# sijieaaa/AGPlace

Measured on AMD Instinct MI355X. Metric: aerial-ground pairs/sec (backbone+ODE+pool), higher is better.
Workload: dtype f16 (fp16 x fp16, fp32 accumulate); 1 GPU; nuScenes-AG 6-cam (C3/C4): MM.forward_q on [b,3,224,1344] + DBVanilla2D on [b,1,3,224,224], ResNet18 stem+layer1-3, euler h=0.1 x3 FCODE, GeM, stage-2 fusion; inference forward; the voxel branch's pooled outputs enter as fixed tensors (SURVEY.md 8d); global_batch=64, parallelism=dp1, bn=per-rank (eval: running statistics), paired_trunks=True, hipgraph=True, steps_in_flight=2, library_default_precision=4, headline_is_library_default=True, streams=2, query_sub_batches_on_streams=1, query_input=fp32 normalised panorama

## Files before the change

### agplace_amd/_lib.py

```python
import ctypes as C
import os

_HERE = os.path.dirname(os.path.abspath(__file__))
LIB_PATH = os.environ.get("AGP_HIP_LIB") or os.path.join(_HERE, "lib", "libagplace_hip.so")

AGP_OK = 0
PREC_BF16 = 1
PREC_F16W2 = 2
PREC_BF16X3 = 3
PREC_F16 = 4
FMT_BF16, FMT_F16 = 0, 1
ACT = {None: 0, "id": 0, "relu": 1, "tanh": 2, "sigmoid": 3}
ODE = {"euler": 0, "midpoint": 1, "rk4": 2}
ODE_ADAPTIVE = {"dopri5": 3}
ODE_STATUS = {0: "ok", 1: "odeint_max_steps attempted steps did not reach t = 1", 2: "step size underflow (t + dt == t)",
              3: "the error ratio is NaN"}
ODE_MAX_STEPS_LIMIT = 4096
E_UNSUPPORTED = 3
GP_FLOATS = 1 + 16384 + 1
_ERR = {1: "AGP_E_BADARG (unsupported shape / enum / null pointer)",
        2: "AGP_E_LAUNCH (HIP launch failed)",
        3: "AGP_E_UNSUPPORTED"}


# ... 60 lines not shown
    "agp_resize_pack_u8_cams": (_I, [_P, _I, _I, _I, _I, _I, _I, _P, _P, _P, _P, C.POINTER(_F), C.POINTER(_F), _I, _P, _P, _P]),
    "agp_center_crop_origin": (_I, [_I, _I, _I, C.POINTER(_I), C.POINTER(_I)]),
    "agp_resize_u8_cams_roi": (_I, [_P, _I, _I, _L, _L, _I, _I, _I, _I, _I, _I, _P, _P, _P, _P, _P, _P]),
    "agp_resize_pack_u8_cams_roi": (_I, [_P, _I, _I, _L, _L, _I, _I, _I, _I, _I, _I, _P, _P, _P, _P, C.POINTER(_F), C.POINTER(_F), _I,
                                         _P, _P, _P]),
    "agp_jitter_u8_cams": (_I, [_P, _I, _I, _I, _I, _P, _P, _P, _P]),
    "agp_jitter_pack_u8_cams": (_I, [_P, _I, _I, _I, _I, _P, _P, C.POINTER(_F), C.POINTER(_F), _I, _P, _P, _P]),
    "agp_unpack_nhwc_to_f32": (_I, [_P, _P, _I, _I, _I, _I, _I, _P, _P]),
    "agp_map_zero_halo": (_I, [_P, _P, _I, _I, _I, _I, _I, _P]),
    "agp_map_absmax": (_I, [_P, _P, _I, _I, _I, _I, _I, _P, _P]),
    "agp_map_absmax_reset": (_I, [_P, _I, _P]),
    "agp_conv2d_fwd": (_I, [C.POINTER(ConvDesc), _P]),
    "agp_conv2d_fwd_grouped": (_I, [C.POINTER(ConvDesc), _I, _P]),
    "agp_conv2d_s2_fwd": (_I, [C.POINTER(ConvDesc), _I, _P]),
    "agp_conv2d_fwd_grouped2": (_I, [C.POINTER(ConvDesc), C.POINTER(ConvStream2), _I, _P]),
    "agp_bblock64_fwd_grouped": (_I, [C.POINTER(BBlock64Desc), _I, _P]),
    "agp_bblock64_pool_floats": (_L, [C.POINTER(BBlock64Desc)]),
    "agp_bblock64_pool_finish": (_I, [_P, _I, _I, _I, _P, _P]),
    "agp_conv_w_q8_prepare": (_I, [_P, _I, _I, _P, C.POINTER(C.c_int32), _P]),
    "agp_conv2d_tile_plan": (_I, [C.POINTER(ConvDesc), _I, C.POINTER(C.c_int32)]),
    "agp_conv2d_stat_tiles": (_I, [C.POINTER(ConvDesc)]),
    "agp_conv2d_pool_blocks": (_I, [C.POINTER(ConvDesc)]),
    "agp_pool_from_conv": (_I, [_P, _I, _I, _I, _I, _P, _P, _P, _P]),
    "agp_bn_stats_from_partial": (_I, [_P, _I, _I, _L, _F, _F, _P, _P, _P, _P, _P, _P, _P, _P, _P]),
    "agp_stem_pool_fwd": (_I, [C.POINTER(ConvDesc), _P]),
    "agp_stem_pool_raw_fwd": (_I, [C.POINTER(ConvDesc), _I, _L, _L, _L, _L, _I, C.POINTER(_F), C.POINTER(_F), _P]),
    "agp_maxpool3x3s2_fwd": (_I, [_P, _P, _I, _I, _I, _I, _I, _P, _P, _I, _I, _I, _P, _P]),
    "agp_bcast_add_fwd": (_I, [_P, _P, _P, _I, _I, _I, _I, _I, _P, _P, _I, _P]),
    "agp_pool_workspace_floats": (_L, [_I, _I, _I, _I]),
    "agp_pool_fwd": (_I, [_P, _P, _I, _I, _I, _I, _I, _P, _F, _P, _P, _P, _P]),
# ... 117 lines not shown
```

### agplace_amd/csrc/conv_dispatch.hip

```cpp
#include "conv_internal.hpp"
using namespace agp_igemm;

static bool fits_31(int n, int h, int w, int c) { return (int64_t)n * (h + 2) * (w + 2) * c * 2 < (1ll << 31); }

static bool conv_3x3s1(const agp_conv_desc* d) {
    return d->kh == 3 && d->kw == 3 && d->stride == 1 && d->pad == 1 && d->in_w_step == d->cin;
}
static bool conv_kxr_ok(const agp_conv_desc* d) {
    return conv_3x3s1(d) && d->pin == 1 && d->pout == 1 && d->hout == d->hin && d->wout == d->win && fits_31(d->n, d->hin, d->win, d->cin);
}

static bool kxr2_member_ok(const agp_conv_desc* d, const agp_conv_desc* d0) {
    return d->in_hi && d->w_hi && d->out_hi && !d->in_lo && !d->out_lo && !d->res_lo && d->n > 0 &&
           d->cin % 32 == 0 && d->cout % 64 == 0 && conv_kxr_ok(d) && agp_internal_use_kxr2(d) &&
           d->cin == d0->cin && d->cout == d0->cout;
}

static bool s2_conv_ok(const agp_conv_desc* c, const agp_conv_desc* d0) {
    return c->prec == AGP_PREC_F16 && c->in_hi && c->w_hi && c->out_hi && !c->in_lo && !c->out_lo && !c->res_hi &&
           !c->stat_partial && !c->pool_partial &&
           c->kh == 3 && c->kw == 3 && c->stride == 2 && c->pad == 1 && c->pin == 1 && c->pout == 1 && c->in_w_step == c->cin &&
           c->hout == (c->hin - 1) / 2 + 1 && c->wout == (c->win - 1) / 2 + 1 &&
           c->cin % 32 == 0 && c->cout % 64 == 0 && c->n > 0 && c->cin == d0->cin && c->cout == d0->cout &&
           fits_31(c->n, c->hin, c->win, c->cin) && fits_31(c->n, c->hout, c->wout, c->cout);
}
static bool s2_downsample_ok(const agp_conv_desc* d, const agp_conv_desc* c) {
    return d->prec == AGP_PREC_F16 && d->w_hi && d->out_hi && !d->in_lo && !d->out_lo && !d->res_hi && !d->stat_partial && !d->pool_partial &&
           d->kh == 1 && d->kw == 1 && d->stride == 2 && d->pad == 0 && d->pin == 1 && d->pout == 1 && d->in_w_step == d->cin &&
// ... 227 lines not shown
    KxrwStreams ds = {};
    const int rc = conv_fill_group(descs, n, ps, true);
    if (rc != AGP_OK) return rc;
    for (int i = 0; i < n; ++i) {
        const agp_conv_stream2* t = s2 + i;
        if (!t->in_hi) continue;
        const int wp = t->win + 2, hp = t->hin + 2;
        KxrwStream& k = ds.s[i];
        k.x = t->in_hi; k.w = t->w_cm;
        k.x_bytes = (uint32_t)((int64_t)t->n * hp * wp * t->cin * 2);
        k.w_bytes = (uint32_t)((int64_t)t->cin * descs[i].cout * 2);
        k.sn = hp * wp * t->cin; k.sh = 2 * wp * t->cin; k.sw = 2 * t->cin; k.base = (wp - 1) * t->cin;
        k.nc = t->cin / 32;
    }
    return agp_internal_conv_kxrw(ps, n, (hipStream_t)stream, nullptr, any ? &ds : nullptr);
}

static int stem_pool_impl(const agp_conv_desc* d, int kind, int64_t sn, int64_t sc, int64_t sh, int64_t sw, int ncam,
                          const float* mean3, const float* std3, void* stream) {
    if (!d || !d->in_hi || !d->w_hi || !d->out_hi || d->in_lo || d->out_lo || d->res_hi) return AGP_E_BADARG;
    if (d->prec != AGP_PREC_F16W2 && d->prec != AGP_PREC_F16) return AGP_E_BADARG;
    if (d->prec == AGP_PREC_F16W2 && !d->w_lo) return AGP_E_BADARG;
    if (d->cin != 32 || d->in_w_step != 4 || d->kw != 1 || d->kh != 7 || d->stride != 2 || d->pad != 3 || d->pin != 3 ||
        d->cout != 64 || !d->relu || d->n <= 0)
        return AGP_E_BADARG;
    const int h1 = (d->hin + 2 * 3 - 7) / 2 + 1, w1 = (d->win + 2 * 3 - 7) / 2 + 1;
    const int h2 = (h1 + 2 - 3) / 2 + 1, w2 = (w1 + 2 - 3) / 2 + 1;
    if (d->hout != h2 || d->wout != w2) return AGP_E_BADARG;
    IgemmParams p = {};
    const int hp = d->hin + 6, wp = d->win + 6;
// ... 30 lines not shown
```

### agplace_amd/csrc/igemm_kxrw.hip

```cpp

#include <type_traits>

#include "conv_internal.hpp"

namespace agp_igemm {

struct KxrwGroup {
    IgemmParams p[KXRW_MAXP];
    int mt_end[KXRW_MAXP];
    int nprob, MT, NT, mt_chunk;
    int MT_full, half_bid0;
    uint32_t* rflag;
    uint32_t r_bytes[KXRW_MAXP];
};
constexpr uint32_t KXRW_ROOB = 0xffffff00u;
__device__ __forceinline__ const KxrwStreams& kxrw_streams(const KxrwStreams& s) { return s; }

constexpr int KW_ROWB = 64;
template <int TM_, int TN_> struct KwShape {
    static constexpr int BM = 128 * TM_, BN = 32 * TN_, BMX = BM + 16;
    static constexpr int XBUF = BMX * KW_ROWB, WTAP = BN * KW_ROWB;
    static constexpr int LDS = 2 * XBUF + 3 * WTAP + 2 * BN * 4;
    static constexpr int STRIP = 32 * 2 * BN, XWAVES = XBUF / STRIP, SPARE = LDS + (TM_ == 1 ? 2048 : 0);
    static constexpr int EPI_LDS = SPARE + (4 - XWAVES) * STRIP;
// ... 397 lines not shown
#pragma unroll
                for (int e = 0; e < 8; ++e) v[e] += r[e];
            }
            rg.any8(v);
            outv[jj] = pack8_h_lo(v, relu_lo);
        }
#pragma unroll
        for (int jj = 0; jj < TN * 2; ++jj) *(u32x4*)(strip + a_off + ((jj ^ a_swz) << 5)) = outv[jj];
        __builtin_amdgcn_fence(__ATOMIC_RELEASE, "wavefront");
        u32x4 lines[NEI];
#pragma unroll
        for (int i = 0; i < NEI; ++i) lines[i] = *(const u32x4*)(strip + l_off + i * 1024);
        if constexpr (TM == 2) {
            if (tm == 0 && RES == 1) wait_vm_lgkm<0>();
        }
#pragma unroll
        for (int i = 0; i < NEI; ++i) {
            const int off = eoff[tm * NEI + i];
            if (off >= 0) *(u32x4*)(ohi + off) = lines[i];
        }
        if constexpr (POOL) {
            if (ppart) {
#pragma unroll
                for (int i = 0; i < NEI; ++i)
                    if (eoff[tm * NEI + i] < 0) *(u32x4*)(strip + l_off + i * 1024) = u32x4{0u, 0u, 0u, 0u};
                __builtin_amdgcn_fence(__ATOMIC_RELEASE, "wavefront");
                auto sweep = [&](auto STAT) {
#pragma clang fp contract(off)
                    constexpr int stat = decltype(STAT)::value;
#pragma unroll
                    for (int p8 = 0; p8 < 32; p8 += 8) {
                        uint32_t w[8];
#pragma unroll
                        for (int u = 0; u < 8; ++u) w[u] = *(const uint32_t*)(strip + (p8 + u) * (2 * BN) + ((lane * 4) ^ (((p8 + u) & 15) << 4)));
// ... 148 lines not shown
    return AGP_OK;
}

}

int agp_internal_conv_kxrw(agp_igemm::IgemmParams* ps, int n, hipStream_t s, agp_igemm::TilePlan* plan, const agp_igemm::KxrwStreams* ds) {
    using namespace agp_igemm;
    if (n < 1 || n > KXRW_MAXP || ps[0].N % 128) return AGP_E_BADARG;
    constexpr int bm = KwShape<2, 4>::BM, bn = KwShape<2, 4>::BN;
    KxrwGroup g = {};
    g.nprob = n;
    int mt = 0;
    bool pool = false;
    for (int i = 0; i < n; ++i) {
        if (ps[i].N != ps[0].N || ps[i].CK != ps[0].CK) return AGP_E_BADARG;
        g.p[i] = ps[i];
        mt += (ps[i].M + bm - 1) / bm;
        g.mt_end[i] = mt;
        pool = pool || ps[i].pool_partial != nullptr;
        const int64_t rb = (int64_t)(ps[i].M / (int)ps[i].d_howo.d) * ps[i].o_sn * 2;
        if (ps[i].r_hi && (rb <= 0 || rb > (int64_t)KXRW_ROOB)) return AGP_E_BADARG;
        g.r_bytes[i] = (uint32_t)rb;
    }
    g.MT = mt;
    g.NT = ps[0].N / bn;
    const KxrwPlan k = kxrw_plan(g.MT, g.NT);
    if (plan) {
        *plan = TilePlan{AGP_CONV_KERNEL_KXRW, bm, bn, g.MT, g.NT, k.MT_full, k.half_tiles, k.blocks};
        return AGP_OK;
    }
// ... 19 lines not shown
```

### agplace_amd/models_baseline/dbvanilla2d.py

```python
from typing import List

import torch
import torch.nn as nn

from .. import autograd_ops, ops, range_guard, train_fns
from ..network.image_fe import ImageFE
from ..network.image_pooling import GeM
from ..network_mm.ffns import _PreparedLinear
from ..options import get_options
from ..vecprog import VecProgram


class MLP(nn.Module):
    def __init__(self, input_dim, output_dim):
        super().__init__()
        self.seq = nn.Sequential(
            nn.Linear(input_dim, output_dim),
            nn.LayerNorm(output_dim),
            nn.ReLU(),
            nn.Linear(output_dim, output_dim),
        )
        self._p0, self._p3 = _PreparedLinear(self.seq[0]), _PreparedLinear(self.seq[3])

    def forward(self, x):
# ... 108 lines not shown
                    x = ops.RawFrames(f.reshape(b * ndb, 1, *f.shape[2:]), h, w, crop=crop,
                                      jitter=None if jitter is None else jitter[:, :, i].reshape(b * ndb, ops.JITTER_RECORD))
                else:
                    x = db_map[:, :, i].reshape(b * ndb, c, h, w)
                if u8:
                    x = x.permute(0, 2, 3, 1).unsqueeze(1)
                if train:
                    fe = self.dbimage_fes[j].fe
                    v = train_fns.TrunkFn.apply(train_fns.anchor_of(fe, self.dbimage_pools[j].p), x, fe, self.dbimage_pools[j], train_fns.MapSink(),
                                                prec, False, i if opt.share_dbfe is True else 0)[0]
                else:
                    if trunk_maps is not None and i in trunk_maps:
                        fpool = trunk_maps[i][1]
                    else:
                        fpool = self.final_pool_request(i)
                        self.dbimage_fes[j].forward_maps(x, prec=prec, final_pool=fpool)
                    v, vscale = (fpool.gem, fpool.scale) if fused is not None else (fpool.true_gem(), None)
                if fused is not None:
                    mlp = self.dbimage_mlps[j]
                    fused.linear(0, mlp._p0.get(), v, scale=vscale)
                    fused.layernorm(0, mlp.seq[1], 0, relu=True)
                    fused.linear(2 + i, mlp._p3.get(), 0)
                    if opt.output_l2 is True:
                        fused.l2norm(2 + i, 2 + i)
                    vecs.append(v)
                    continue
                v = self.dbimage_mlps[j](v)
                if opt.output_l2 is True:
                    v = autograd_ops.l2normalize(v)
                vecs.append(v)
            if fused is not None:
# ... 30 lines not shown
```

### agplace_amd/network_mm/image_fe.py

```python
import torch.nn as nn

from .. import range_guard
from ..options import get_options
from ..resnet import ResNet


class ImageFE(nn.Module):
    _ALLOWED = ("resnet18", "resnet34")
    _LAST_DIM = {"resnet18": {2: 128, 3: 256, 4: 512}, "resnet34": {2: 128, 3: 256, 4: 512},
                 "resnet50": {2: 512, 3: 1024, 4: 2048}}

    def __init__(self, fe_type, layers, opt=None):
        super().__init__()
        self.opt = opt
        self.fe_type = fe_type
        layers = [int(x) for x in layers.split('_')]
        self.layers = layers
        if fe_type not in self._ALLOWED or len(layers) not in (2, 3, 4):
            raise NotImplementedError
        self.last_dim = self._LAST_DIM[fe_type][len(layers)]
        self.fe = ResNet(fe_type, nstages=len(layers))

    def forward_maps(self, x, prec=None, level_means=None, final_pool=None):
        if len(self.layers) not in (3, 4):
            raise NotImplementedError
        prec = get_options().mfma_precision if prec is None else prec
        return self.fe.forward_maps(x, prec=prec, level_means=level_means, final_pool=final_pool)

    def export_precision(self):
        p = get_options().mfma_precision
        return 2 if p == 4 else p

    def forward(self, x, prec=None):
        prec = self.export_precision() if prec is None else prec
        with range_guard.guarded(self, self.opt or get_options(), prec, self.training):
            maps = self.forward_maps(x, prec=prec)
            x_list = [m.to_f32() for m in maps]
        return x_list[-1], x_list

    def poll_fp16_range(self):
        range_guard.poll(self)

# ... 3 lines not shown
```

### agplace_amd/network_mm/mm.py

```python
import torch
import torch.nn as nn

from .. import autograd_ops, ops, range_guard, sparse, train_fns
from ..options import get_options
from .ffns import _PreparedLinear
from .fuse_block_toshallow import FuseBlockToShallow
from ..vecprog import VecProgram, VecProgramUnfit
from .image_fe import ImageFE
from .image_pooling import GeM
from .stage2fuse_blockadd import Stage2FuseBlockAdd


class MM(nn.Module):
    def __init__(self, drop=None, opt=None):
        super().__init__()
        self.opt = opt = opt or get_options()
        self.drop = drop
        self.image_fe = ImageFE(fe_type=opt.mm_imgfe, layers=opt.mm_imgfe_layers)
        self.image_fe.fe.set_image_norm(opt.image_mean, opt.image_std)
        self.image_pool = GeM()
        planes = [int(x) for x in opt.mm_voxfe_planes.split('_')]
        layers = [int(x) for x in opt.mm_voxfe_layers.split('_')]
        self.vox_fe = sparse.MinkFPN(in_channels=1, out_channels=planes[-1], planes=planes, layers=layers,
                                     num_top_down=opt.mm_voxfe_ntd, conv0_kernel_size=5, block=sparse.ECABasicBlock)
# ... 294 lines not shown
            vp.linear(2, s2._prep_fuseimg[0].get(exp=-e3), 1)
            fv_img = vp.store(2)
        elif e3:
            vp.wsum(2, [1], [ops.pow2_scalar(dev, -e3)])
            fv_img = vp.store(2)
        if sparse_vox and s2._prep_fusevox[0] is not None:
            vp.linear(3, s2._prep_fusevox[0].get(), 1)
            fv_vox = vp.store(3)
        if rider and vp.fits_beside(rider[0]):
            vp.run(rider=rider.pop())
        else:
            vp.run()
        m = s2._ws.map("add0", imagefeatmap.n, imagefeatmap.h, imagefeatmap.w, imagefeatmap.c, 1, prec, dev)
        ops.bcast_add(imagefeatmap, fv_img, m)
        s2pool = ops.PoolReq(s2.poolimage.p, eps=s2.poolimage.eps, want_mean=True, want_gem=True, gem_out=out_rows.get('stg2imagevec'))
        imap = s2.ffnsimg[0].forward_map(m, prec, pool=s2pool)
        mean, stg2imagevec, s2scale = s2pool.mean, s2pool.gem, s2pool.scale
        if sparse_vox:
            vm = sparse.modules.seg_affine(voxmap, add=fv_vox)
            vm = s2.ffnsvox[0](vm, prec=prec)
            stg2voxvec = s2.poolvox(vm)
            vf = s2.projsvoxfuse[0][0](vm, prec=prec) if opt.stg2_useproj is True else vm
            voxvec_fuse = sparse.modules.global_avg_pool(vf)
        else:
            stg2voxvec, voxvec_fuse = data_dict['stg2voxvec'].float(), data_dict['voxvec_fuse'].float()
        vt = VecProgram(b, dev)
        if s2._prep_imgfuse[0] is not None:
            vt.linear(0, s2._prep_imgfuse[0].get(), mean, scale=s2scale)
        else:
            vt.load(0, mean, s2scale)
        vt.load(1, fusevec)
# ... 108 lines not shown
```

### agplace_amd/network_mm/stage2fuse_blockadd.py

```python
import torch
import torch.nn as nn

from .. import autograd_ops, ops, sparse, train_fns, train_graph
from ..options import get_options
from .ffns import _PreparedLinear
from .image_pooling import GeM


class _Conv1x1AsLinear:

    def __init__(self, conv):
        self.conv = conv

    @property
    def weight(self):
        return self.conv.weight.view(self.conv.out_channels, self.conv.in_channels)

    @property
    def bias(self):
        return self.conv.bias


class _PreparedConv1x1(_PreparedLinear):
    def __init__(self, conv):
# ... 23 lines not shown
        self._ws = ops.Workspace()
        self._units = None
        self._map_exp = {}

    def _prepared(self, e_io=0, e_mid=0):
        key = tuple((t.data_ptr(), t._version) for t in list(self.parameters()) + list(self.buffers())) + (e_io, e_mid)
        if key != self._key:
            cws = []
            for conv, bn, e_in, e_out in ((self.conv1, self.bn1, e_io, e_mid), (self.conv2, self.bn2, e_mid, e_io)):
                s, t = ops.fold_exp(*ops.fold_bn(bn.weight, bn.bias, bn.running_mean, bn.running_var, bn.eps,
                                                 conv_bias=conv.bias), e_in, e_out)
                cws.append(ops.ConvWeights(conv.weight, s, t, 1, 1))
            self._cw, self._key = cws, key
        return self._cw

    def forward_map(self, x: ops.SplitMap, prec=3, pool=None):
        e_mid = int(self._map_exp.get("conv1", 0)) if prec != 3 else 0
        c1, c2 = self._prepared(x.exp, e_mid)
        dev = x.hi.device
        t = self._ws.map("t", x.n, x.h, x.w, x.c, 1, prec, dev)
        o = self._ws.map("o", x.n, x.h, x.w, x.c, 1, prec, dev)
        t.exp, o.exp = e_mid, x.exp
        ops.probe_map(self, "in", x)
        ops.conv2d(x, c1, t, relu=True, prec=prec)
        ops.probe_map(self, "conv1", t)
        ops.conv2d(t, c2, o, residual=x, relu=True, prec=prec, pool=pool)
        ops.probe_map(self, "out", o)
        return o

    def forward(self, x, prec=3):
        if isinstance(x, ops.SplitMap):
            return self.forward_map(x, prec)
        xm = ops.pack_f32(x, x.shape[1], 1, prec)
        return self.forward_map(xm, prec).to_f32()

    def forward_map_train(self, x: ops.SplitMap, prec=3):
        if self._units is None:
# ... 169 lines not shown
```

### agplace_amd/ops.py

```python
import ctypes as C
import math
import os

import torch

from . import _lib
from ._lib import ptr, check

GEM_EPS = 1e-6
CONV_PROFILE = None
LO_FP8 = True
CHUNK_MAJOR_TRAIN = True
USE_W_CM = True


def _L():
    return _lib.load()


def _need_cuda(t, what):
    if not t.is_cuda:
        raise RuntimeError(f"{what}: tensor must live on the GPU (agplace_amd has no CPU path)")


# ... 87 lines not shown

def probe_map(owner, name, m):
    if MAP_PROBE is not None:
        MAP_PROBE(owner, name, m)


def map_absmax(m: SplitMap, word):
    check(_L().agp_map_absmax(ptr(m.hi), ptr(m.lo), m.n, m.h, m.w, m.c, m.pad, ptr(word), _lib.stream()), "agp_map_absmax")


def absmax_reset(words):
    check(_L().agp_map_absmax_reset(ptr(words), words.numel(), _lib.stream()), "agp_map_absmax_reset")


def count_saturated(m: SplitMap):
    if m.lo is not None:
        return 0
    return int((m.hi.view(torch.float16).abs() >= 65504).sum().item())


class Workspace:

    def __init__(self):
        self.bufs = {}

    def map(self, tag, n, h, w, c, pad, prec, device, h16=False):
        key = (tag, n, h, w, c, pad, prec, str(device), torch.cuda.current_stream(device).cuda_stream)
        m = self.bufs.get(key)
        if m is None:
            m = SplitMap.alloc(n, h, w, c, pad, prec, device)
            self.bufs[key] = m
# ... 437 lines not shown
    jobs = [tuple(j) + (None,) * (6 - len(j)) for j in jobs]
    arr = (_lib.ConvDesc * len(jobs))()
    for d, (x, cw, out, residual, relu, pool) in zip(arr, jobs):
        _fill_conv_desc(d, x, cw, out, residual, relu, prec)
        if pool is not None and x.lo is None and out.lo is None and int(_L().agp_conv2d_pool_blocks(C.byref(d))) > 0:
            d.pool_partial = 1
    if len(jobs) == 1:
        if stat_partial:
            arr[0].stat_partial = 1
        if hi_only:
            arr[0].hi_only = 1
        return tile_plan(arr[0])
    return tile_plan(arr)


class PoolReq:
    __slots__ = ("p", "eps", "want_mean", "want_gem", "mean", "gem", "fused", "_partial", "gem_out", "exp")

    def __init__(self, p=None, eps=GEM_EPS, want_mean=True, want_gem=False, gem_out=None):
        if want_gem and p is None:
            raise ValueError("PoolReq: GeM needs its exponent tensor p")
        self.p = None if p is None else p.detach()
        self.eps, self.want_mean, self.want_gem = eps, want_mean, want_gem
        self.mean = self.gem = self._partial = None
        self.gem_out = gem_out
        self.fused = False
        self.exp = 0

    @property
    def scale(self):
        t = self.mean if self.mean is not None else self.gem
        return pow2_scalar(t.device, self.exp)

    def true_mean(self):
        return scale_pow2(self.mean, self.exp)

    def true_gem(self):
        return scale_pow2(self.gem, self.exp)

    def attach(self, d, x, cw, out, prec):
        self.fused = False
        self.exp = out.exp
        if x.lo is None and out.lo is None:
            blocks = int(_L().agp_conv2d_pool_blocks(C.byref(d)))
            if blocks > 0:
                self._partial = torch.empty(blocks * 2 * cw.cout, dtype=torch.float32, device=out.hi.device)
                d.pool_partial = ptr(self._partial)
                d.pool_p = ptr(self.p) if self.want_gem else None
                d.pool_eps = math.ldexp(self.eps, -self.exp)
                self.fused = True

    def finish(self, out):
        go = self.gem_out
        if go is not None and (tuple(go.shape) != (out.n, out.c) or go.dtype != torch.float32 or not go.is_contiguous()):
            go = None
        self.exp = out.exp
        if not self.fused:
            self.mean, self.gem = pool_map(out, self.p, want_mean=self.want_mean, want_gem=self.want_gem, eps=self.eps, gem_out=go,
                                           raw=True)
            return
        dev = out.hi.device
        self.mean = torch.empty((out.n, out.c), dtype=torch.float32, device=dev) if self.want_mean else None
        self.gem = (go if go is not None else torch.empty((out.n, out.c), dtype=torch.float32, device=dev)) if self.want_gem else None
        check(_L().agp_pool_from_conv(ptr(self._partial), out.n, out.h, out.w, out.c, ptr(self.p) if self.want_gem else None,
                                      ptr(self.mean), ptr(self.gem), _lib.stream()), "agp_pool_from_conv")


class SqStatReq:
    __slots__ = ("fused", "partial", "blocks")

    def __init__(self):
        self.fused, self.partial, self.blocks = False, None, 0

    def attach(self, d, x, cw, out, prec):
        self.fused = False
        if x.lo is None and out.lo is None:
# ... 44 lines not shown
            if c2 is not None:
                d.w_cm, d.w_cm_lo = ptr(c2[0]), ptr(c2[1])
    if LO_FP8 and prec == _lib.PREC_F16W2:
        q = cw.q8()
        if q is not None:
            d.w_q8, d.w_q8_exp = ptr(q[0]), q[1]
    return d


def conv2d_grouped(jobs, prec):
    jobs = [tuple(j) + (None,) * (6 - len(j)) for j in jobs]
    if len(jobs) == 1:
        x, cw, out, residual, relu, pool = jobs[0]
        return [conv2d(x, cw, out, residual=residual, relu=relu, prec=prec, pool=pool)]
    arr = (_lib.ConvDesc * len(jobs))()
    keep = []
    for d, (x, cw, out, residual, relu, pool) in zip(arr, jobs):
        keep.append(cw.planes(prec))
        _fill_conv_desc(d, x, cw, out, residual, relu, prec)
        if pool is not None:
            pool.attach(d, x, cw, out, prec)
    e0 = e1 = None
    if CONV_PROFILE is not None:
        e0, e1 = torch.cuda.Event(enable_timing=True), torch.cuda.Event(enable_timing=True)
        e0.record()
    check(_L().agp_conv2d_fwd_grouped(arr, len(jobs), _lib.stream()), "agp_conv2d_fwd_grouped")
    if CONV_PROFILE is not None:
        e1.record()
        x, cw, out = jobs[0][:3]
        macs = sum(j[0].n * j[2].h * j[2].w * j[1].cout * j[1].alg_k for j in jobs)
        CONV_PROFILE.append((e0, e1, macs, (sum(j[0].n for j in jobs), out.h, out.w, cw.cin, cw.cout, cw.kh, cw.kw, cw.stride)))
    for j in jobs:
        if j[5] is not None:
            j[5].finish(j[2])
    return [j[2] for j in jobs]


class Stream2Weights:
    __slots__ = ("cin", "cout", "plane", "shift", "fusable")

    def __init__(self, weight, scale, shift):
# ... 29 lines not shown
            if x2.lo is not None or x2.pad != 1 or x2.c != sw.cin or sw.plane is None:
                raise ValueError("conv2d_grouped2: the second stream is a one-plane fp16 map with a 1-pixel halo and fusable weights")
            t.in_hi, t.w_cm = ptr(x2.hi), ptr(sw.plane)
            t.n, t.hin, t.win, t.cin = x2.n, x2.h, x2.w, sw.cin
    check(_L().agp_conv2d_fwd_grouped2(arr, st, len(jobs), _lib.stream()), "agp_conv2d_fwd_grouped2")
    return [j[2] for j in jobs]


def conv2d(x: SplitMap, cw: ConvWeights, out: SplitMap, residual: SplitMap = None, relu=False, prec=3, stat_partial=None, pool=None,
           bstat=None, hi_only=False):
    d = _fill_conv_desc(_lib.ConvDesc(), x, cw, out, residual, relu, prec, stat_partial, bstat)
    if hi_only:
        d.hi_only = 1
    if pool is not None:
        pool.attach(d, x, cw, out, prec)
    if CONV_PROFILE is not None:
        e0, e1 = torch.cuda.Event(enable_timing=True), torch.cuda.Event(enable_timing=True)
        e0.record()
        check(_L().agp_conv2d_fwd(C.byref(d), _lib.stream()), "agp_conv2d_fwd")
        e1.record()
        CONV_PROFILE.append((e0, e1, x.n * out.h * out.w * cw.cout * cw.alg_k,
                             (x.n, out.h, out.w, cw.cin, cw.cout, cw.kh, cw.kw, cw.stride)))
    else:
        check(_L().agp_conv2d_fwd(C.byref(d), _lib.stream()), "agp_conv2d_fwd")
    if pool is not None:
        pool.finish(out)
    return out


FUSED_BLOCK64 = True


def bblock64_ok(x: SplitMap, cw1: ConvWeights, cw2: ConvWeights, prec):
    if not FUSED_BLOCK64 or prec != _lib.PREC_F16 or x.lo is not None or x.pad != 1 or x.c != 64 or x.h % 2:
        return False
    for cw in (cw1, cw2):
        if (cw.cin, cw.cout, cw.kh, cw.kw, cw.stride, cw.pad) != (64, 64, 3, 3, 1, 1) or cw.in_w_step_stem or cw.w is None:
            return False
    return x.n * (x.h + 2) * (x.w + 2) * 128 < (1 << 31)
# ... 466 lines not shown
```

### agplace_amd/pair.py

```python
import torch


from . import ops, range_guard, resnet

RIDER = True


def can_pair(modelq, modeldb, qdata, dbdata):
    if modelq.training or modeldb.training or torch.is_grad_enabled():
        return False
    fq, fdbs = modelq.image_fe.fe, [m.fe for m in modeldb.dbimage_fes]
    db_map = dbdata['db_map']
    nmap = db_map.shape[-4]
    if modelq.opt.mfma_precision != modeldb.opt.mfma_precision or db_map.dim() not in (5, 6):
        return False
    if modeldb.opt.share_dbfe is True and nmap > 1:
        return False
    return all((f.fe_type, f.nstages) == (fq.fe_type, fq.nstages) for f in fdbs[:nmap])


def _resized_tiles(modelq, modeldb, qdata, dbdata):
    if 'query_jitter' in qdata and 'query_frames' not in qdata:
        raise ValueError("embed_pair: `query_jitter` (colour jitter records) needs `query_frames`")
    if 'db_jitter' in dbdata and 'db_frames' not in dbdata:
# ... 43 lines not shown
    b = img.shape[0]
    if k > 1 and 'coords' not in qdata and 'points' not in qdata and b % k == 0 and b >= 2 * k and db_map.shape[0] % k == 0:
        return _embed_pair_substreams(modelq, modeldb, qdata, dbdata, k)
    return _embed_pair_one(modelq, modeldb, qdata, dbdata)


def _embed_pair_one(modelq, modeldb, qdata, dbdata, q_rows=None, db_rows=None):
    opt = modelq.opt
    prec = opt.mfma_precision
    image = modelq.query_image(qdata)
    db_map = dbdata['db_map']
    u8 = db_map.dtype == torch.uint8
    if db_map.dim() == 5:
        db_map = db_map.unsqueeze(1)
    nets, xs, lms, fps = [modelq.image_fe.fe], [image], [[]], [modelq.final_pool_request()]
    nmap = db_map.shape[2]
    for i in range(nmap):
        nets.append(modeldb.dbimage_fes[i].fe)
        if u8:
            bb, ndb, _, h, w, _ = db_map.shape
            xs.append(db_map[:, :, i].reshape(bb * ndb, 1, h, w, 3))
        else:
            bb, ndb, _, c, h, w = db_map.shape
            xs.append(db_map[:, :, i].reshape(bb * ndb, c, h, w))
        lms.append(None)
        fps.append(modeldb.final_pool_request(i))
    maps = resnet.forward_maps_multi(nets, xs, prec=prec, level_means=lms, final_pools=fps)
    head = [] if RIDER else None
    out_db = modeldb.forward_db(dbdata, trunk_maps={i: (maps[1 + i], fps[1 + i]) for i in range(nmap)}, out_rows=db_rows,
                                defer_head=head)
    out_q = modelq.forward_q(qdata, image_maps=(maps[0], lms[0], fps[0]), out_rows=q_rows, rider=head)
    if head:
        head.pop().run()
    return out_q, out_db


def _slice(d, b, lo, hi):
    out = {}
    for name, v in d.items():
        if torch.is_tensor(v) and v.dim() > 0 and v.shape[0] == b:
            out[name] = v[lo:hi]
        elif isinstance(v, (list, tuple)) and all(torch.is_tensor(t) and t.shape[0] == b for t in v):
# ... 82 lines not shown
```

### agplace_amd/resnet.py

```python
import math

import os

import torch
import torch.nn as nn

from . import ops, train_graph

ARCH = {
    "resnet18": ("basic", [2, 2, 2, 2]),
    "resnet34": ("basic", [3, 4, 6, 3]),
    "resnet50": ("bottleneck", [3, 4, 6, 3]),
}
PLANES = [64, 128, 256, 512]


def _conv(cin, cout, k, stride, pad):
    m = nn.Conv2d(cin, cout, k, stride, pad, bias=False)
    nn.init.kaiming_normal_(m.weight, mode="fan_out", nonlinearity="relu")
    return m


class _Block(nn.Module):
    def __init__(self, kind, inplanes, planes, stride):
# ... 167 lines not shown
                raise ValueError("stem input map must be NHWC4 with halo 3 in the conv's storage format")
            return ops.slice_map(x, lo, hi)
        raw = isinstance(x, ops.RawFrames)
        want16 = h16 and prec == 3 and not raw and x.dtype != torch.uint8
        xin = ops.slice_map(self._ws.map(tag, n, h, w, 4, 3, prec, dev, h16=want16), lo, hi)
        if not want16 and xin.h16 is not None:
            xin = ops.SplitMap(xin.hi, xin.lo, xin.n, xin.h, xin.w, xin.c, xin.pad)
        if raw:
            x.stem_map(lo, hi, prec, self.image_mean, self.image_std, xin)
        elif x.dtype == torch.uint8:
            ops.pack_cameras_u8(x[lo:hi], prec, self.image_mean, self.image_std, out=xin)
        else:
            xin = ops.pack_f32(x[lo:hi], 4, 3, prec, out=xin)
        return xin

    def forward_maps(self, x, prec=3, level_means=None, final_pool=None):
        return forward_maps_multi([self], [x], prec=prec, level_means=[level_means], final_pools=[final_pool])[0]

    def _unit(self, name, conv, bn, stem=False, pre="t."):
        u = self._units.get(pre + name)
        if u is None:
            u = train_graph.ConvBNUnit(conv, bn, pre + name, self._ws, stem=stem)
            self._units[pre + name] = u
        return u

    def forward_maps_train(self, x, prec=3, slot=0):
        if not hasattr(self, "_units"):
            self._units, self._tapes, self._tape_gens = {}, {}, {}
        self._tape_gens[slot] = self._tape_gens.get(slot, 0) + 1
        pre = "t." if slot == 0 else f"t{slot}."
        n, h, w, dev = self._input_geometry(x)
        ws = self._ws
# ... 79 lines not shown
                pnext = None
            if added:
                g, part = gh, pnext
            else:
                acc = ws.map(units[0].tag + ".gsum", gh.n, gh.h, gh.w, gh.c, 1, prec, dev)
                g, part = train_graph.map_add(gh, gx2, acc), None
        if g is not None:
            stem.backward(g, need_gx=False, pool_argmax=argmax, pooled=s)


STEM_READS_INPUT = "auto"
SATURATION_CHECK = True
STAGE1_CHUNK = 1 << 30


def forward_maps_multi(nets, xs, prec=3, level_means=None, final_pools=None):
    R = len(nets)
    level_means = level_means or [None] * R
    final_pools = final_pools or [None] * R
    stage_pool = [{} for _ in range(R)]
    a = nets[0]
    for b in nets[1:]:
        if (b.fe_type, b.nstages) != (a.fe_type, a.nstages):
            raise ValueError("forward_maps_multi: the trunks must share one architecture")
    preps = [net._prepared(scaled=prec != 3) for net in nets]
    fuses = [net._prepared_fuse(scaled=prec != 3) for net in nets]
    geo = [net._input_geometry(x) for net, x in zip(nets, xs)]
    devs = [g[3] for g in geo]
    nchunks = max(1, -(-geo[0][0] // STAGE1_CHUNK))
    for r in range(R):
        for li in range(a.nstages):
            last_stage = li == a.nstages - 1
            if last_stage and final_pools[r] is not None:
                stage_pool[r][li] = final_pools[r]
            elif not last_stage and level_means[r] is not None:
                stage_pool[r][li] = ops.PoolReq(want_mean=True, want_gem=False)

    def run_stage(li, cur, lo, hi):
        act = [r for r in range(R) if hi[r] > lo[r]]
        nblocks = len(getattr(a, f"layer{li + 1}"))
        for bi in range(nblocks):
            blks = {r: getattr(nets[r], f"layer{li + 1}")[bi] for r in act}
            cws = {r: preps[r][(li, bi)] for r in act}
            idt = dict(cur)

            def view(r, tag, h_, w_, c_, e_):
                v = ops.slice_map(nets[r]._ws.map(tag, geo[r][0], h_, w_, c_, 1, prec, devs[r]), lo[r], hi[r])
                v.exp = e_
                return v
            mexp = {r: preps[r]["exp"] for r in act}
            lname = f"layer{li + 1}.{bi}"
# ... 53 lines not shown
                    for r in act:
                        pool = stage_pool[r].get(li)
                        if pool is not None:
                            pool.fused = False
                            pool.finish(o2[r])
                cur = o2
                continue
            for ci in range(nconv):
                last = ci == nconv - 1
                jobs = []
                for r in act:
                    cw = cws[r][0][ci]
                    oh = ops.conv_out_size(t[r].h, cw.kh, cw.stride, cw.pad)
                    ow = ops.conv_out_size(t[r].w, cw.kw, cw.stride, cw.pad)
                    pool = stage_pool[r].get(li) if (last and bi == nblocks - 1 and (li > 0 or nchunks == 1)) else None
                    jobs.append((t[r], cw, view(r, f"c{li}.{bi}.{ci}", oh, ow, cw.cout, mexp[r][(li, bi, ci)]), idt[r] if last else None,
                                 True, pool))
                if ci == 0 and ds_jobs:
                    if len(jobs) + len(ds_jobs) <= 4 and not (cws[act[0]][0][0].kh == 3 and cws[act[0]][0][0].stride == 1):
                        outs_ = ops.conv2d_grouped(jobs + ds_jobs, prec)[:len(jobs)]
                    else:
                        ops.conv2d_grouped(ds_jobs, prec)
                        outs_ = ops.conv2d_grouped(jobs, prec)
                else:
                    outs_ = ops.conv2d_grouped(jobs, prec)
                t = {r: o for r, o in zip(act, outs_)}
                if ops.MAP_PROBE is not None:
                    for r in act:
                        ops.probe_map(nets[r], f"{lname}.out" if last else f"{lname}.conv{ci + 1}", t[r])
                        if ci == 0 and ds_jobs:
                            ops.probe_map(nets[r], f"{lname}.downsample", idt[r])
            cur = t
# ... 69 lines not shown
```

### include/agplace_hip.h

```cpp
#ifndef AGPLACE_HIP_H
#define AGPLACE_HIP_H

#include <stdint.h>

#ifdef __cplusplus
extern "C" {
#endif

#define AGP_OK 0
#define AGP_E_BADARG 1
#define AGP_E_LAUNCH 2
#define AGP_E_UNSUPPORTED 3

#define AGP_PREC_BF16 1
#define AGP_PREC_F16W2 2
#define AGP_PREC_BF16X3 3
#define AGP_PREC_F16 4

#define AGP_FMT_BF16 0
#define AGP_FMT_F16 1

#define AGP_ACT_ID 0
#define AGP_ACT_RELU 1
#define AGP_ACT_TANH 2
// ... 89 lines not shown
    uint32_t* out_absmax;
    int32_t pool_stat;
    int32_t reserved0;
} agp_conv_desc;
int agp_conv2d_fwd(const agp_conv_desc* d, void* stream);

int agp_conv2d_fwd_grouped(const agp_conv_desc* descs, int n, void* stream);

typedef struct agp_conv_stream2 {
    const void* in_hi;
    const void* w_cm;
    int32_t n, hin, win, cin;
} agp_conv_stream2;
int agp_conv2d_s2_fwd(const agp_conv_desc* descs, int n, void* stream);
int agp_conv2d_fwd_grouped2(const agp_conv_desc* descs, const agp_conv_stream2* s2, int n, void* stream);

#define AGP_CONV_KERNEL_GENERIC 1
#define AGP_CONV_KERNEL_DIRECT_X 2
#define AGP_CONV_KERNEL_KXR 3
#define AGP_CONV_KERNEL_KXR2 4
#define AGP_CONV_KERNEL_KXRW 5
#define AGP_CONV_KERNEL_S2 6
int agp_conv2d_tile_plan(const agp_conv_desc* descs, int n, int32_t plan[8]);

int agp_conv2d_stat_tiles(const agp_conv_desc* d);

int agp_conv2d_pool_blocks(const agp_conv_desc* d);
int agp_pool_from_conv(const float* partial, int n, int h, int w, int c, const float* p, float* mean_out,
                       float* gem_out, void* stream);

// ... 283 lines not shown
```

Measured before the change: 43020 pairs/s.

## Skip storing final conv maps when only their pooled epilogue output is consumed

Adds a grouped conv entry point that lets a pooling-epilogue conv skip writing its output map to global memory. It is used for the last-stage convs of the DB image trunks and for the stage-2 image FFN, whose maps are only consumed through GeM/mean pooling. This removes a large fp16 store of the last-stage and stage-2 maps and the workspace that holds them. In exchange, the saturation check and map probes are not possible on those maps, so they fall back to a stored map when a check or probe is due.

```diff
diff --git a/agplace_amd/_lib.py b/agplace_amd/_lib.py
--- a/agplace_amd/_lib.py
+++ b/agplace_amd/_lib.py
@@ -98,6 +98,7 @@
     "agp_conv2d_fwd_grouped": (_I, [C.POINTER(ConvDesc), _I, _P]),
     "agp_conv2d_s2_fwd": (_I, [C.POINTER(ConvDesc), _I, _P]),
     "agp_conv2d_fwd_grouped2": (_I, [C.POINTER(ConvDesc), C.POINTER(ConvStream2), _I, _P]),
+    "agp_conv2d_fwd_grouped_nomap": (_I, [C.POINTER(ConvDesc), C.POINTER(C.c_int32), _I, _P]),
     "agp_bblock64_fwd_grouped": (_I, [C.POINTER(BBlock64Desc), _I, _P]),
     "agp_bblock64_pool_floats": (_L, [C.POINTER(BBlock64Desc)]),
     "agp_bblock64_pool_finish": (_I, [_P, _I, _I, _I, _P, _P]),
diff --git a/agplace_amd/csrc/conv_dispatch.hip b/agplace_amd/csrc/conv_dispatch.hip
--- a/agplace_amd/csrc/conv_dispatch.hip
+++ b/agplace_amd/csrc/conv_dispatch.hip
@@ -10,8 +10,8 @@
     return conv_3x3s1(d) && d->pin == 1 && d->pout == 1 && d->hout == d->hin && d->wout == d->win && fits_31(d->n, d->hin, d->win, d->cin);
 }
 
-static bool kxr2_member_ok(const agp_conv_desc* d, const agp_conv_desc* d0) {
-    return d->in_hi && d->w_hi && d->out_hi && !d->in_lo && !d->out_lo && !d->res_lo && d->n > 0 &&
+static bool kxr2_member_ok(const agp_conv_desc* d, const agp_conv_desc* d0, bool need_out = true) {
+    return d->in_hi && d->w_hi && (d->out_hi || !need_out) && !d->in_lo && !d->out_lo && !d->res_lo && d->n > 0 &&
            d->cin % 32 == 0 && d->cout % 64 == 0 && conv_kxr_ok(d) && agp_internal_use_kxr2(d) &&
            d->cin == d0->cin && d->cout == d0->cout;
 }
@@ -269,6 +269,23 @@
         k.nc = t->cin / 32;
     }
     return agp_internal_conv_kxrw(ps, n, (hipStream_t)stream, nullptr, any ? &ds : nullptr);
+}
+
+extern "C" int agp_conv2d_fwd_grouped_nomap(const agp_conv_desc* descs, const int32_t* no_map, int n, void* stream) {
+    if (!descs || !no_map) return AGP_E_BADARG;
+    if (n < 1 || n > 4 || AGP_TUNE("CONV_KERNEL", 0) || !AGP_TUNE("KXR_WIDE", 1)) return AGP_E_UNSUPPORTED;
+    for (int i = 0; i < n; ++i) {
+        const agp_conv_desc* d = descs + i;
+        if (!kxr2_member_ok(d, descs, false) || d->w_lo || d->hi_only || d->cout % 128) return AGP_E_UNSUPPORTED;
+        if (!no_map[i] && !d->out_hi) return AGP_E_BADARG;
+        if (no_map[i] && (!d->pool_partial || agp_conv2d_pool_blocks(d) <= 0)) return AGP_E_UNSUPPORTED;
+    }
+    IgemmParams ps[4];
+    const int rc = conv_fill_group(descs, n, ps, true);
+    if (rc != AGP_OK) return rc;
+    for (int i = 0; i < n; ++i)
+        if (no_map[i]) ps[i].o_hi = nullptr;
+    return agp_internal_conv_kxrw(ps, n, (hipStream_t)stream, nullptr, nullptr);
 }
 
 static int stem_pool_impl(const agp_conv_desc* d, int kind, int64_t sn, int64_t sc, int64_t sh, int64_t sw, int ncam,
diff --git a/agplace_amd/csrc/igemm_kxrw.hip b/agplace_amd/csrc/igemm_kxrw.hip
--- a/agplace_amd/csrc/igemm_kxrw.hip
+++ b/agplace_amd/csrc/igemm_kxrw.hip
@@ -435,10 +435,12 @@
         if constexpr (TM == 2) {
             if (tm == 0 && RES == 1) wait_vm_lgkm<0>();
         }
-#pragma unroll
-        for (int i = 0; i < NEI; ++i) {
-            const int off = eoff[tm * NEI + i];
-            if (off >= 0) *(u32x4*)(ohi + off) = lines[i];
+        if (!POOL || ohi) {
+#pragma unroll
+            for (int i = 0; i < NEI; ++i) {
+                const int off = eoff[tm * NEI + i];
+                if (off >= 0) *(u32x4*)(ohi + off) = lines[i];
+            }
         }
         if constexpr (POOL) {
             if (ppart) {
@@ -617,6 +619,7 @@
     bool pool = false;
     for (int i = 0; i < n; ++i) {
         if (ps[i].N != ps[0].N || ps[i].CK != ps[0].CK) return AGP_E_BADARG;
+        if (!ps[i].o_hi && !ps[i].pool_partial) return AGP_E_BADARG;
         g.p[i] = ps[i];
         mt += (ps[i].M + bm - 1) / bm;
         g.mt_end[i] = mt;
diff --git a/agplace_amd/models_baseline/dbvanilla2d.py b/agplace_amd/models_baseline/dbvanilla2d.py
--- a/agplace_amd/models_baseline/dbvanilla2d.py
+++ b/agplace_amd/models_baseline/dbvanilla2d.py
@@ -146,7 +146,7 @@
                         fpool = trunk_maps[i][1]
                     else:
                         fpool = self.final_pool_request(i)
-                        self.dbimage_fes[j].forward_maps(x, prec=prec, final_pool=fpool)
+                        self.dbimage_fes[j].forward_maps(x, prec=prec, final_pool=fpool, keep_last=False)
                     v, vscale = (fpool.gem, fpool.scale) if fused is not None else (fpool.true_gem(), None)
                 if fused is not None:
                     mlp = self.dbimage_mlps[j]
diff --git a/agplace_amd/network_mm/image_fe.py b/agplace_amd/network_mm/image_fe.py
--- a/agplace_amd/network_mm/image_fe.py
+++ b/agplace_amd/network_mm/image_fe.py
@@ -21,11 +21,11 @@
         self.last_dim = self._LAST_DIM[fe_type][len(layers)]
         self.fe = ResNet(fe_type, nstages=len(layers))
 
-    def forward_maps(self, x, prec=None, level_means=None, final_pool=None):
+    def forward_maps(self, x, prec=None, level_means=None, final_pool=None, keep_last=True):
         if len(self.layers) not in (3, 4):
             raise NotImplementedError
         prec = get_options().mfma_precision if prec is None else prec
-        return self.fe.forward_maps(x, prec=prec, level_means=level_means, final_pool=final_pool)
+        return self.fe.forward_maps(x, prec=prec, level_means=level_means, final_pool=final_pool, keep_last=keep_last)
 
     def export_precision(self):
         p = get_options().mfma_precision
diff --git a/agplace_amd/network_mm/mm.py b/agplace_amd/network_mm/mm.py
--- a/agplace_amd/network_mm/mm.py
+++ b/agplace_amd/network_mm/mm.py
@@ -332,7 +332,7 @@
         m = s2._ws.map("add0", imagefeatmap.n, imagefeatmap.h, imagefeatmap.w, imagefeatmap.c, 1, prec, dev)
         ops.bcast_add(imagefeatmap, fv_img, m)
         s2pool = ops.PoolReq(s2.poolimage.p, eps=s2.poolimage.eps, want_mean=True, want_gem=True, gem_out=out_rows.get('stg2imagevec'))
-        imap = s2.ffnsimg[0].forward_map(m, prec, pool=s2pool)
+        s2.ffnsimg[0].forward_map(m, prec, pool=s2pool, keep_out=False)
         mean, stg2imagevec, s2scale = s2pool.mean, s2pool.gem, s2pool.scale
         if sparse_vox:
             vm = sparse.modules.seg_affine(voxmap, add=fv_vox)
diff --git a/agplace_amd/network_mm/stage2fuse_blockadd.py b/agplace_amd/network_mm/stage2fuse_blockadd.py
--- a/agplace_amd/network_mm/stage2fuse_blockadd.py
+++ b/agplace_amd/network_mm/stage2fuse_blockadd.py
@@ -61,13 +61,16 @@
             self._cw, self._key = cws, key
         return self._cw
 
-    def forward_map(self, x: ops.SplitMap, prec=3, pool=None):
+    def forward_map(self, x: ops.SplitMap, prec=3, pool=None, keep_out=True):
         e_mid = int(self._map_exp.get("conv1", 0)) if prec != 3 else 0
         c1, c2 = self._prepared(x.exp, e_mid)
         dev = x.hi.device
         t = self._ws.map("t", x.n, x.h, x.w, x.c, 1, prec, dev)
-        o = self._ws.map("o", x.n, x.h, x.w, x.c, 1, prec, dev)
-        t.exp, o.exp = e_mid, x.exp
+        t.exp = e_mid
+        o = ops.map_shape(x.n, x.h, x.w, x.c, 1, x.exp)
+        if keep_out or pool is None or not ops.pooled_only_ok(t, c2, o, prec):
+            o = self._ws.map("o", x.n, x.h, x.w, x.c, 1, prec, dev)
+            o.exp = x.exp
         ops.probe_map(self, "in", x)
         ops.conv2d(x, c1, t, relu=True, prec=prec)
         ops.probe_map(self, "conv1", t)
diff --git a/agplace_amd/ops.py b/agplace_amd/ops.py
--- a/agplace_amd/ops.py
+++ b/agplace_amd/ops.py
@@ -125,7 +125,7 @@
 
 
 def count_saturated(m: SplitMap):
-    if m.lo is not None:
+    if m.lo is not None or m.hi is None:
         return 0
     return int((m.hi.view(torch.float16).abs() >= 65504).sum().item())
 
@@ -593,10 +593,35 @@
     return tile_plan(arr)
 
 
+POOLED_ONLY_NO_MAP = True
+
+
+def map_shape(n, h, w, c, pad, exp=0):
+    return SplitMap(None, None, n, h, w, c, pad, exp=exp)
+
+
+def pooled_only_ok(x: SplitMap, cw: ConvWeights, out: SplitMap, prec):
+    return bool(POOLED_ONLY_NO_MAP and MAP_PROBE is None and prec == _lib.PREC_F16 and x.lo is None and cw.cout % 128 == 0
+                and int(_L().agp_conv2d_pool_blocks(C.byref(conv_desc(x, cw, out, prec)))) > 0)
+
+
+def _no_map(out, pool, what):
+    no = out.hi is None or (pool is not None and getattr(pool, "no_map", False))
+    if no and (pool is None or not pool.fused):
+        raise RuntimeError(f"{what}: a conv that stores no map must pool in its epilogue (ops.pooled_only_ok)")
+    return no
+
+
+def _launch_no_map(arr, flags):
+    n = len(flags)
+    check(_L().agp_conv2d_fwd_grouped_nomap(arr, (C.c_int32 * n)(*[int(f) for f in flags]), n, _lib.stream()), "agp_conv2d_fwd_grouped_nomap")
+
+
 class PoolReq:
-    __slots__ = ("p", "eps", "want_mean", "want_gem", "mean", "gem", "fused", "_partial", "gem_out", "exp")
-
-    def __init__(self, p=None, eps=GEM_EPS, want_mean=True, want_gem=False, gem_out=None):
+    __slots__ = ("p", "eps", "want_mean", "want_gem", "mean", "gem", "fused", "_partial", "gem_out", "exp", "no_map")
+
+    def __init__(self, p=None, eps=GEM_EPS, want_mean=True, want_gem=False, gem_out=None, no_map=False):
+        self.no_map = no_map
         if want_gem and p is None:
             raise ValueError("PoolReq: GeM needs its exponent tensor p")
         self.p = None if p is None else p.detach()
@@ -623,7 +648,7 @@
         if x.lo is None and out.lo is None:
             blocks = int(_L().agp_conv2d_pool_blocks(C.byref(d)))
             if blocks > 0:
-                self._partial = torch.empty(blocks * 2 * cw.cout, dtype=torch.float32, device=out.hi.device)
+                self._partial = torch.empty(blocks * 2 * cw.cout, dtype=torch.float32, device=x.hi.device)
                 d.pool_partial = ptr(self._partial)
                 d.pool_p = ptr(self.p) if self.want_gem else None
                 d.pool_eps = math.ldexp(self.eps, -self.exp)
@@ -638,7 +663,7 @@
             self.mean, self.gem = pool_map(out, self.p, want_mean=self.want_mean, want_gem=self.want_gem, eps=self.eps, gem_out=go,
                                            raw=True)
             return
-        dev = out.hi.device
+        dev = self._partial.device
         self.mean = torch.empty((out.n, out.c), dtype=torch.float32, device=dev) if self.want_mean else None
         self.gem = (go if go is not None else torch.empty((out.n, out.c), dtype=torch.float32, device=dev)) if self.want_gem else None
         check(_L().agp_pool_from_conv(ptr(self._partial), out.n, out.h, out.w, out.c, ptr(self.p) if self.want_gem else None,
@@ -713,17 +738,21 @@
         x, cw, out, residual, relu, pool = jobs[0]
         return [conv2d(x, cw, out, residual=residual, relu=relu, prec=prec, pool=pool)]
     arr = (_lib.ConvDesc * len(jobs))()
-    keep = []
+    keep, flags = [], []
     for d, (x, cw, out, residual, relu, pool) in zip(arr, jobs):
         keep.append(cw.planes(prec))
         _fill_conv_desc(d, x, cw, out, residual, relu, prec)
         if pool is not None:
             pool.attach(d, x, cw, out, prec)
+        flags.append(_no_map(out, pool, "conv2d_grouped"))
     e0 = e1 = None
     if CONV_PROFILE is not None:
         e0, e1 = torch.cuda.Event(enable_timing=True), torch.cuda.Event(enable_timing=True)
         e0.record()
-    check(_L().agp_conv2d_fwd_grouped(arr, len(jobs), _lib.stream()), "agp_conv2d_fwd_grouped")
+    if any(flags):
+        _launch_no_map(arr, flags)
+    else:
+        check(_L().agp_conv2d_fwd_grouped(arr, len(jobs), _lib.stream()), "agp_conv2d_fwd_grouped")
     if CONV_PROFILE is not None:
         e1.record()
         x, cw, out = jobs[0][:3]
@@ -783,15 +812,22 @@
         d.hi_only = 1
     if pool is not None:
         pool.attach(d, x, cw, out, prec)
+    no_map = _no_map(out, pool, "conv2d")
+
+    def launch():
+        if no_map:
+            _launch_no_map(C.byref(d), [1])
+        else:
+            check(_L().agp_conv2d_fwd(C.byref(d), _lib.stream()), "agp_conv2d_fwd")
     if CONV_PROFILE is not None:
         e0, e1 = torch.cuda.Event(enable_timing=True), torch.cuda.Event(enable_timing=True)
         e0.record()
-        check(_L().agp_conv2d_fwd(C.byref(d), _lib.stream()), "agp_conv2d_fwd")
+        launch()
         e1.record()
         CONV_PROFILE.append((e0, e1, x.n * out.h * out.w * cw.cout * cw.alg_k,
                              (x.n, out.h, out.w, cw.cin, cw.cout, cw.kh, cw.kw, cw.stride)))
     else:
-        check(_L().agp_conv2d_fwd(C.byref(d), _lib.stream()), "agp_conv2d_fwd")
+        launch()
     if pool is not None:
         pool.finish(out)
     return out
diff --git a/agplace_amd/pair.py b/agplace_amd/pair.py
--- a/agplace_amd/pair.py
+++ b/agplace_amd/pair.py
@@ -81,6 +81,7 @@
     if db_map.dim() == 5:
         db_map = db_map.unsqueeze(1)
     nets, xs, lms, fps = [modelq.image_fe.fe], [image], [[]], [modelq.final_pool_request()]
+    keep = [True]
     nmap = db_map.shape[2]
     for i in range(nmap):
         nets.append(modeldb.dbimage_fes[i].fe)
@@ -92,7 +93,8 @@
             xs.append(db_map[:, :, i].reshape(bb * ndb, c, h, w))
         lms.append(None)
         fps.append(modeldb.final_pool_request(i))
-    maps = resnet.forward_maps_multi(nets, xs, prec=prec, level_means=lms, final_pools=fps)
+        keep.append(False)
+    maps = resnet.forward_maps_multi(nets, xs, prec=prec, level_means=lms, final_pools=fps, keep_last=keep)
     head = [] if RIDER else None
     out_db = modeldb.forward_db(dbdata, trunk_maps={i: (maps[1 + i], fps[1 + i]) for i in range(nmap)}, out_rows=db_rows,
                                 defer_head=head)
diff --git a/agplace_amd/resnet.py b/agplace_amd/resnet.py
--- a/agplace_amd/resnet.py
+++ b/agplace_amd/resnet.py
@@ -205,8 +205,8 @@
             xin = ops.pack_f32(x[lo:hi], 4, 3, prec, out=xin)
         return xin
 
-    def forward_maps(self, x, prec=3, level_means=None, final_pool=None):
-        return forward_maps_multi([self], [x], prec=prec, level_means=[level_means], final_pools=[final_pool])[0]
+    def forward_maps(self, x, prec=3, level_means=None, final_pool=None, keep_last=True):
+        return forward_maps_multi([self], [x], prec=prec, level_means=[level_means], final_pools=[final_pool], keep_last=[keep_last])[0]
 
     def _unit(self, name, conv, bn, stem=False, pre="t."):
         u = self._units.get(pre + name)
@@ -316,8 +316,9 @@
 STAGE1_CHUNK = 1 << 30
 
 
-def forward_maps_multi(nets, xs, prec=3, level_means=None, final_pools=None):
+def forward_maps_multi(nets, xs, prec=3, level_means=None, final_pools=None, keep_last=None):
     R = len(nets)
+    keep_last = keep_last or [True] * R
     level_means = level_means or [None] * R
     final_pools = final_pools or [None] * R
     stage_pool = [{} for _ in range(R)]
@@ -337,6 +338,9 @@
                 stage_pool[r][li] = final_pools[r]
             elif not last_stage and level_means[r] is not None:
                 stage_pool[r][li] = ops.PoolReq(want_mean=True, want_gem=False)
+
+    capturing = torch.cuda.is_current_stream_capturing()
+    sat_due = [SATURATION_CHECK and prec != 3 and not capturing and net.__dict__.get("_sat_checked") != net._prep_key for net in nets]
 
     def run_stage(li, cur, lo, hi):
         act = [r for r in range(R) if hi[r] > lo[r]]
@@ -420,8 +424,12 @@
                     oh = ops.conv_out_size(t[r].h, cw.kh, cw.stride, cw.pad)
                     ow = ops.conv_out_size(t[r].w, cw.kw, cw.stride, cw.pad)
                     pool = stage_pool[r].get(li) if (last and bi == nblocks - 1 and (li > 0 or nchunks == 1)) else None
-                    jobs.append((t[r], cw, view(r, f"c{li}.{bi}.{ci}", oh, ow, cw.cout, mexp[r][(li, bi, ci)]), idt[r] if last else None,
-                                 True, pool))
+                    e_out = mexp[r][(li, bi, ci)]
+                    out_ = ops.map_shape(hi[r] - lo[r], oh, ow, cw.cout, 1, e_out)
+                    if not (pool is not None and li == a.nstages - 1 and li > 0 and not keep_last[r] and not sat_due[r]
+                            and ops.pooled_only_ok(t[r], cw, out_, prec)):
+                        out_ = view(r, f"c{li}.{bi}.{ci}", oh, ow, cw.cout, e_out)
+                    jobs.append((t[r], cw, out_, idt[r] if last else None, True, pool))
                 if ci == 0 and ds_jobs:
                     if len(jobs) + len(ds_jobs) <= 4 and not (cws[act[0]][0][0].kh == 3 and cws[act[0]][0][0].stride == 1):
                         outs_ = ops.conv2d_grouped(jobs + ds_jobs, prec)[:len(jobs)]
diff --git a/include/agplace_hip.h b/include/agplace_hip.h
--- a/include/agplace_hip.h
+++ b/include/agplace_hip.h
@@ -127,6 +127,8 @@
 } agp_conv_stream2;
 int agp_conv2d_s2_fwd(const agp_conv_desc* descs, int n, void* stream);
 int agp_conv2d_fwd_grouped2(const agp_conv_desc* descs, const agp_conv_stream2* s2, int n, void* stream);
+
+int agp_conv2d_fwd_grouped_nomap(const agp_conv_desc* descs, const int32_t* no_map, int n, void* stream);
 
 #define AGP_CONV_KERNEL_GENERIC 1
 #define AGP_CONV_KERNEL_DIRECT_X 2
```

After: 43250 pairs/s, median of 5. Within noise of the previous version (+0.5%).
